# Sbte/RAILS

Measured on AMD Instinct MI355X. Metric: RAILS iterations/sec (+ A*V SpMM HBM GB/s in roofline), m=1M rows/GPU, k=128, fp64, higher is better.
Workload: dtype f64

## Files before the change

### include/rails_hip.h

```cpp
#ifndef RAILS_HIP_H
#define RAILS_HIP_H

#include <stddef.h>
#include <stdint.h>

#ifdef __cplusplus
extern "C" {
#endif

#define RAILS_OK 0
#define RAILS_EINVAL -1
#define RAILS_EHIP -2
#define RAILS_ENOMEM -3
#define RAILS_ELAPACK -4
#define RAILS_ECOMM -5
#define RAILS_ENODEV -6

typedef struct rails_ctx rails_ctx;
typedef struct rails_csr rails_csr;
typedef struct rails_panel rails_panel;

const char *rails_last_error(void);
const char *rails_version(void);

// ... 85 lines not shown

typedef struct rails_sweep_plan rails_sweep_plan;
int rails_sweep_plan_create(int64_t m, int64_t ncols, const int64_t *rowptr, const int32_t *col, const double *val,
                            const int *params, rails_sweep_plan **out);
int rails_sweep_plan_destroy(rails_sweep_plan *plan);
int rails_sweep_plan_info(const rails_sweep_plan *plan, int64_t *iinfo, double *dinfo);
int rails_sweep_plan_array(const rails_sweep_plan *plan, int which, const void **ptr, int64_t *count);


int rails_panel_create(rails_ctx *ctx, int64_t m_local, int capacity, rails_panel **out);
int rails_panel_create_ld(rails_ctx *ctx, int64_t m_local, int capacity, int ld, rails_panel **out);
int rails_panel_destroy(rails_panel *P);
int64_t rails_panel_rows(const rails_panel *P);
int rails_panel_capacity(const rails_panel *P);
int rails_panel_ld(const rails_panel *P);
void *rails_panel_device_ptr(const rails_panel *P);
int rails_panel_reserve(rails_ctx *ctx, rails_panel *P, int capacity);

int rails_panel_upload(rails_ctx *ctx, rails_panel *P, int c0, int nc, const double *host, int64_t ldh);
int rails_panel_download(rails_ctx *ctx, const rails_panel *P, int c0, int nc, double *host, int64_t ldh);

int rails_panel_fill(rails_ctx *ctx, rails_panel *P, int c0, int nc, double value);
int rails_panel_scale(rails_ctx *ctx, rails_panel *P, int c0, int nc, double s);
int rails_panel_copy(rails_ctx *ctx, const rails_panel *X, int xc0, int nc, rails_panel *Y, int yc0);
int rails_panel_axpy(rails_ctx *ctx, double alpha, const rails_panel *X, int xc0, int nc, rails_panel *Y,
                     int yc0);
int rails_panel_random(rails_ctx *ctx, rails_panel *P, int c0, int nc);

int rails_gram(rails_ctx *ctx, const rails_panel *X, int xc0, int a, const rails_panel *Y, int yc0, int b,
               double *C_host, int ldc);

int rails_panel_gemm(rails_ctx *ctx, double alpha, const rails_panel *X, int xc0, int k, const double *C_host,
                     int ldc, int r, double beta, rails_panel *Y, int yc0);

int rails_ctx_enable_library_gemm(rails_ctx *ctx);
int rails_ctx_library_gemm_ready(const rails_ctx *ctx);

int rails_deferred_reserve(rails_ctx *ctx, int nslots, int64_t doubles_per_slot);
int rails_gram_deferred(rails_ctx *ctx, const rails_panel *X, int xc0, int a, const rails_panel *Y, int yc0, int b, int slot);
int rails_panel_gemm_deferred(rails_ctx *ctx, double alpha, const rails_panel *X, int xc0, int k, int slot, int ld, int r, double beta,
                              rails_panel *Y, int yc0);
int rails_chol_inverse_deferred(rails_ctx *ctx, int slot_in, int w, int slot_out);
int rails_update_gram_deferred(rails_ctx *ctx, double alpha, const rails_panel *X, int xc0, int k, const double *C_host, int ldc, int r,
                               rails_panel *Y, int yc0, int r2, int slot);
int rails_update_gram_deferred_out(rails_ctx *ctx, double alpha, const rails_panel *X, int xc0, int k, const double *C_host, int ldc, int r,
                                   const rails_panel *Y, int yc0, rails_panel *Yout, int oc0, int r2, int slot);
int rails_deferred_fetch(rails_ctx *ctx, int slot, int64_t n, double *host_out);

int rails_panel_gemm_wide(rails_ctx *ctx, double alpha, const rails_panel *X, int xc0, int k, const double *C_host, int ldc, int r,
                          double beta, rails_panel *Y, int yc0);

void rails_dense_set_tile_fit(int on);
int rails_dense_tile_fit(void);
int rails_dense_last_tiles(const rails_ctx *ctx, int *update_gram_nbw, int *gram_cols_ti, int *gemm_wide_tr);

int rails_orthogonalize(rails_ctx *ctx, rails_panel *V, int k_old, int w, int method, int *used);
int rails_orthogonalize_deflated(rails_ctx *ctx, rails_panel *V, int k_old, int w, const rails_panel *N, int nc0, int q, int method, int *used);

int rails_panel_colnorms2(rails_ctx *ctx, const rails_panel *X, int c0, int nc, double *out_host);

int rails_orthogonalize_range(rails_ctx *ctx, rails_panel *V, int k_old, int w, const rails_panel *N, int nc0, int q, double tol, int *kept,
                              int32_t *kept_idx);

int rails_resid_lanczos(rails_ctx *ctx, const rails_panel *AV, int avc0, const rails_panel *MV, int mvc0, int k,
                        const double *T_host, int ldt, const rails_panel *B, int bc0, int p, int L,
                        double *H_host, int ldh, int *steps);

int rails_resid_lanczos_sparse(rails_ctx *ctx, const rails_panel *AV, int avc0, const rails_panel *MV, int mvc0, int k, const double *T_host,
                               int ldt, const rails_sprhs *S, int L, double *H_host, int ldh, int *steps);

int rails_lanczos_start(rails_ctx *ctx, const rails_panel *AV, int avc0, const rails_panel *MV, int mvc0, int k,
                        const rails_panel *B, int bc0, int p, double *sums_host);

int rails_lanczos_vectors(rails_ctx *ctx, const double *S_host, int lds, int w, rails_panel *Out, int oc0);
int rails_lanczos_last_launch(rails_ctx *ctx, int *nch, int *unroll, int *nblocks);
int rails_lanczos_release(rails_ctx *ctx);

int rails_ctx_reserve_staging(rails_ctx *ctx, size_t bytes);
int rails_timer_start(rails_ctx *ctx);
int rails_timer_stop(rails_ctx *ctx, double *ms);


void rails_sb03md(char dico, char job, char fact, char trans, int n, double *A, int lda, double *X, int ldx,
                  double *scale, int *info);
void rails_sb03md_counts(long *smith, long *schur);
void rails_sb03md_adi_counts(long *extended, long *fresh);
void rails_sb03md_set_pause(int calls);
void rails_dsyev(char jobz, char uplo, int n, double *a, int lda, double *w, int *info);
void rails_dsteqr(char compz, int n, double *d, double *e, double *z, int ldz, double *work, int *info);
void rails_dgemm(char transa, char transb, int m, int n, int k, double alpha, const double *A, int lda, const double *B,
                 int ldb, double beta, double *C, int ldc);
void rails_dtrsm(char side, char uplo, char transa, char diag, int m, int n, double alpha, const double *A, int lda, double *B, int ldb);
void rails_dpotrf(char uplo, int n, double *a, int lda, int *info);
void rails_dpstrf(char uplo, int n, double *a, int lda, int *piv, int *rank, double tol, int *info);
void rails_range_basis(int m, int n, double *a, int lda, double tol, double *q, int ldq, int *rank, int *info);
int rails_host_lapack_init(const char *path);
const char *rails_host_lapack_path(void);

#ifdef __cplusplus
}
#endif
#endif
```

### rails_amd/_lib.py

```python
import ctypes as C
import os

_HERE = os.path.dirname(os.path.abspath(__file__))
LIB_PATH = os.path.join(_HERE, "lib", "librails_hip.so")

_dp = C.POINTER(C.c_double)
_ip = C.POINTER(C.c_int)
_i64p = C.POINTER(C.c_int64)
_i32p = C.POINTER(C.c_int32)
_vp = C.c_void_p

ALLREDUCE_FN = C.CFUNCTYPE(C.c_int, C.c_void_p, C.c_void_p, C.c_size_t, C.c_void_p)
HALO_FN = C.CFUNCTYPE(C.c_int, C.c_void_p, C.c_void_p, C.c_void_p, C.c_int, C.c_void_p)
APPLY_FN = C.CFUNCTYPE(C.c_int, C.c_void_p, C.c_int, C.c_void_p, C.c_int, C.c_int, C.c_void_p, C.c_int)

SIGNATURES = {
    "rails_last_error": (C.c_char_p, []),
    "rails_version": (C.c_char_p, []),
    "rails_ctx_create": (C.c_int, [C.c_int, _vp, C.POINTER(_vp)]),
    "rails_ctx_destroy": (C.c_int, [_vp]),
    "rails_ctx_sync": (C.c_int, [_vp]),
    "rails_ctx_stream": (_vp, [_vp]),
    "rails_ctx_set_meter": (C.c_int, [_vp, C.c_int]),
    "rails_ctx_enable_library_gemm": (C.c_int, [_vp]),
# ... 27 lines not shown
    "rails_csr_sweep_stats": (C.c_int, [_vp, C.c_int, _dp]),
    "rails_csr_tile_stats": (C.c_int, [_vp, _dp]),
    "rails_csr_prepare": (C.c_int, [_vp, _vp, C.c_int, C.c_int, C.POINTER(C.c_int)]),
    "rails_csr_last_kernel": (C.c_char_p, [_vp]),
    "rails_sweep_plan_create": (C.c_int, [C.c_int64, C.c_int64, _i64p, _i32p, _dp, _ip, C.POINTER(_vp)]),
    "rails_sweep_plan_destroy": (C.c_int, [_vp]),
    "rails_sweep_plan_info": (C.c_int, [_vp, _i64p, _dp]),
    "rails_sweep_plan_array": (C.c_int, [_vp, C.c_int, C.POINTER(_vp), _i64p]),
    "rails_panel_create": (C.c_int, [_vp, C.c_int64, C.c_int, C.POINTER(_vp)]),
    "rails_panel_create_ld": (C.c_int, [_vp, C.c_int64, C.c_int, C.c_int, C.POINTER(_vp)]),
    "rails_panel_destroy": (C.c_int, [_vp]),
    "rails_panel_rows": (C.c_int64, [_vp]),
    "rails_panel_capacity": (C.c_int, [_vp]),
    "rails_panel_ld": (C.c_int, [_vp]),
    "rails_panel_device_ptr": (_vp, [_vp]),
    "rails_panel_reserve": (C.c_int, [_vp, _vp, C.c_int]),
    "rails_panel_upload": (C.c_int, [_vp, _vp, C.c_int, C.c_int, _dp, C.c_int64]),
    "rails_panel_download": (C.c_int, [_vp, _vp, C.c_int, C.c_int, _dp, C.c_int64]),
    "rails_panel_fill": (C.c_int, [_vp, _vp, C.c_int, C.c_int, C.c_double]),
    "rails_panel_scale": (C.c_int, [_vp, _vp, C.c_int, C.c_int, C.c_double]),
    "rails_panel_copy": (C.c_int, [_vp, _vp, C.c_int, C.c_int, _vp, C.c_int]),
    "rails_panel_axpy": (C.c_int, [_vp, C.c_double, _vp, C.c_int, C.c_int, _vp, C.c_int]),
    "rails_sptrsv_create": (C.c_int, [_vp, C.c_int64, _i64p, _i32p, _dp, C.c_int, C.c_int, C.POINTER(_vp)]),
    "rails_sptrsv_destroy": (None, [_vp]),
    "rails_sptrsv_levels": (C.c_int64, [_vp]),
    "rails_sptrsv_solve": (C.c_int, [_vp, _vp, _vp, C.c_int, C.c_int]),
    "rails_panel_permute_rows": (C.c_int, [_vp, _vp, C.c_int, C.c_int, _vp, C.c_int, _vp, C.c_int]),
    "rails_index_upload": (C.c_int, [_vp, _i32p, C.c_int64, C.POINTER(_vp)]),
    "rails_index_free": (None, [_vp, _vp]),
    "rails_lu_create": (C.c_int, [_vp, C.c_int64, _i64p, _i32p, _dp, _i64p, _i32p, _dp, _i32p, _i32p, _i32p, C.c_int64, C.POINTER(_vp)]),
    "rails_lu_destroy": (None, [_vp]),
    "rails_lu_solve": (C.c_int, [_vp, _vp, C.c_int, _vp, C.c_int, C.c_int, _vp, C.c_int]),
    "rails_lu_stats": (C.c_int, [_vp, _i64p, C.c_int]),
    "rails_csr_create_lu": (C.c_int, [_vp, _vp, C.POINTER(_vp)]),
    "rails_csr_transpose_host": (C.c_int, [C.c_int64, C.c_int64, _i64p, _i32p, _dp, _i64p, _i32p, _dp]),
    "rails_csr_gram_norm2_host": (C.c_int, [C.c_int64, C.c_int64, _i64p, _i32p, _dp, _i64p, _i32p, _dp, _dp]),
    "rails_sprhs_create": (C.c_int, [_vp, C.c_int64, C.c_int, _i64p, _i32p, _dp, C.POINTER(_vp)]),
    "rails_sprhs_destroy": (None, [_vp]),
    "rails_sprhs_rows": (C.c_int64, [_vp]),
    "rails_sprhs_cols": (C.c_int64, [_vp]),
    "rails_sprhs_nnz": (C.c_int64, [_vp]),
    "rails_sprhs_gram_norm2": (C.c_double, [_vp]),
    "rails_sprhs_apply": (C.c_int, [_vp, _vp, C.c_int, _vp, C.c_int, C.c_int, _vp, C.c_int]),
    "rails_csr_create_sprhs": (C.c_int, [_vp, _vp, C.POINTER(_vp)]),
    "rails_csr_cols": (C.c_int64, [_vp]),
    "rails_csr_sprhs": (_vp, [_vp]),
    "rails_resid_lanczos_sparse": (C.c_int, [_vp, _vp, C.c_int, _vp, C.c_int, C.c_int, _dp, C.c_int, _vp, C.c_int, _dp, C.c_int, _ip]),
    "rails_panel_random": (C.c_int, [_vp, _vp, C.c_int, C.c_int]),
    "rails_gram": (C.c_int, [_vp, _vp, C.c_int, C.c_int, _vp, C.c_int, C.c_int, _dp, C.c_int]),
    "rails_panel_gemm": (C.c_int, [_vp, C.c_double, _vp, C.c_int, C.c_int, _dp, C.c_int, C.c_int, C.c_double, _vp, C.c_int]),
    "rails_panel_gemm_wide": (C.c_int, [_vp, C.c_double, _vp, C.c_int, C.c_int, _dp, C.c_int, C.c_int, C.c_double, _vp, C.c_int]),
    "rails_dense_set_tile_fit": (None, [C.c_int]),
    "rails_dense_tile_fit": (C.c_int, []),
    "rails_dense_last_tiles": (C.c_int, [_vp, _ip, _ip, _ip]),
    "rails_orthogonalize": (C.c_int, [_vp, _vp, C.c_int, C.c_int, C.c_int, _ip]),
    "rails_orthogonalize_deflated": (C.c_int, [_vp, _vp, C.c_int, C.c_int, _vp, C.c_int, C.c_int, C.c_int, _ip]),
    "rails_panel_colnorms2": (C.c_int, [_vp, _vp, C.c_int, C.c_int, _dp]),
    "rails_orthogonalize_range": (C.c_int, [_vp, _vp, C.c_int, C.c_int, _vp, C.c_int, C.c_int, C.c_double, _ip, _i32p]),
    "rails_resid_lanczos": (C.c_int, [_vp, _vp, C.c_int, _vp, C.c_int, C.c_int, _dp, C.c_int, _vp, C.c_int, C.c_int, C.c_int,
                                      _dp, C.c_int, _ip]),
    "rails_lanczos_start": (C.c_int, [_vp, _vp, C.c_int, _vp, C.c_int, C.c_int, _vp, C.c_int, C.c_int, _dp]),
    "rails_lanczos_vectors": (C.c_int, [_vp, _dp, C.c_int, C.c_int, _vp, C.c_int]),
    "rails_lanczos_last_launch": (C.c_int, [_vp, _ip, _ip, _ip]),
    "rails_lanczos_release": (C.c_int, [_vp]),
    "rails_timer_start": (C.c_int, [_vp]),
    "rails_timer_stop": (C.c_int, [_vp, _dp]),
    "rails_sb03md": (None, [C.c_char, C.c_char, C.c_char, C.c_char, C.c_int, _dp, C.c_int, _dp, C.c_int, _dp, _ip]),
    "rails_dsyev": (None, [C.c_char, C.c_char, C.c_int, _dp, C.c_int, _dp, _ip]),
    "rails_dsteqr": (None, [C.c_char, C.c_int, _dp, _dp, _dp, C.c_int, _dp, _ip]),
    "rails_ctx_reserve_staging": (C.c_int, [_vp, C.c_size_t]),
    "rails_sb03md_set_pause": (None, [C.c_int]),
    "rails_sb03md_counts": (None, [C.POINTER(C.c_long), C.POINTER(C.c_long)]),
    "rails_sb03md_adi_counts": (None, [C.POINTER(C.c_long), C.POINTER(C.c_long)]),
    "rails_dtrsm": (None, [C.c_char, C.c_char, C.c_char, C.c_char, C.c_int, C.c_int, C.c_double, _dp, C.c_int, _dp, C.c_int]),
    "rails_dgemm": (None, [C.c_char, C.c_char, C.c_int, C.c_int, C.c_int, C.c_double, _dp, C.c_int, _dp, C.c_int, C.c_double, _dp, C.c_int]),
    "rails_dpotrf": (None, [C.c_char, C.c_int, _dp, C.c_int, _ip]),
    "rails_dpstrf": (None, [C.c_char, C.c_int, _dp, C.c_int, _ip, _ip, C.c_double, _ip]),
    "rails_range_basis": (None, [C.c_int, C.c_int, _dp, C.c_int, C.c_double, _dp, C.c_int, _ip, _ip]),
    "rails_host_lapack_init": (C.c_int, [C.c_char_p]),
    "rails_host_lapack_path": (C.c_char_p, []),
}

_lib = None


class RailsError(RuntimeError):
    pass


def load():
    global _lib
    if _lib is not None:
        return _lib
    if not os.path.exists(LIB_PATH):
        raise RailsError(
            "rails_amd: %s is missing -- build it with `python -c 'import __graft_entry__ as g; g.build()'` "
            "or `make -C rails_amd/csrc`; there is no CPU fallback" % LIB_PATH)
    lib = C.CDLL(LIB_PATH, mode=C.RTLD_GLOBAL)
    for name, (res, args) in SIGNATURES.items():
        fn = getattr(lib, name)
        fn.restype = res
        fn.argtypes = args
    try:
        from ._solver_sigs import bind as _bind_solver
        _bind_solver(lib)
    except ImportError:
# ... 13 lines not shown
```

### rails_amd/csrc/dense.hip

```cpp
#include "rails_internal.h"

#include <dlfcn.h>
#include <atomic>
#include <mutex>

#include <algorithm>

namespace {

typedef double v4f64 __attribute__((ext_vector_type(4)));
typedef double v2f64 __attribute__((ext_vector_type(2)));

std::atomic<int> g_tile_fit{-1};

bool dense_tile_fit()
{
    int v = g_tile_fit.load(std::memory_order_relaxed);
    if (v < 0) {
        const char *e = getenv("RAILS_DENSE_TILE_FIT");
        int undecided = -1;
        g_tile_fit.compare_exchange_strong(undecided, (e ? atoi(e) : 1) ? 1 : 0);
        v = g_tile_fit.load(std::memory_order_relaxed);
    }
    return v != 0;
}

__device__ __forceinline__ v4f64 mfma_f64(double a, double b, v4f64 c)
{
    return __builtin_amdgcn_mfma_f64_16x16x4f64(a, b, c, 0, 0, 0);
}

struct OneSeg {
    const double *X;
    int ld;
    struct Row {
        const double *x;
    };
    __device__ int col(int c) const { return c; }
    __device__ Row row(int64_t r) const { return {X + r * ld}; }
    __device__ static const double *at(Row r, int c) { return r.x + c; }
};
struct TwoSeg {
    const double *X1;
    int ld1, a1;
    const double *X2;
    int ld2;
    struct Col {
        int off;
        bool second;
    };
    struct Row {
        const double *x1, *x2;
    };
    __device__ Col col(int c) const
    {
        const bool second = c >= a1;
        return {second ? c - a1 : c, second};
    }
    __device__ Row row(int64_t r) const { return {X1 + r * ld1, X2 + r * ld2}; }
    __device__ static const double *at(Row r, Col c) { return (c.second ? r.x2 : r.x1) + c.off; }
};

template <int TI, int TJ>
__global__ __launch_bounds__(256) __attribute__((amdgpu_waves_per_eu(3, 8))) void k_gram(const double *__restrict__ X, int ldx, int a, const double *__restrict__ Y, int ldy,
                                              int b, int64_t m, int64_t rows_per_slab, int ngj, double *__restrict__ partial)
{
    const OneSeg Xo{X, ldx};
#include "dense_gram.inc"
}

template <int TI, int TJ>
__global__ __launch_bounds__(256) void k_gram2(const double *__restrict__ X1, int ldx1, int a1, const double *__restrict__ X2, int ldx2, int a,
                                               const double *__restrict__ Y, int ldy, int b, int64_t m, int64_t rows_per_slab, int ngj,
                                               double *__restrict__ partial)
{
    const TwoSeg Xo{X1, ldx1, a1, X2, ldx2};
#include "dense_gram.inc"
}

template <int TI, int TJ, int NE = 0>
__global__ __launch_bounds__(256) __attribute__((amdgpu_waves_per_eu(3, 8))) void k_gram_cols(const double *__restrict__ X, int ldx, int a,
                                                                                             const double *__restrict__ Y, int ldy, int b, int64_t m,
                                                                                             int64_t rows_per_slab, double *__restrict__ partial)
{
    const OneSeg Xo{X, ldx};
#include "dense_gram_cols.inc"
}

template <int TI, int TJ, int NE>
__global__ __launch_bounds__(256) void k_gram_cols2(const double *__restrict__ X1, int ldx1, int a1, const double *__restrict__ X2, int ldx2, int a,
                                                    const double *__restrict__ Y, int ldy, int b, int64_t m, int64_t rows_per_slab,
                                                    double *__restrict__ partial)
{
    const TwoSeg Xo{X1, ldx1, a1, X2, ldx2};
#include "dense_gram_cols.inc"
}

__global__ __launch_bounds__(1024) void k_reduce_partials(const double *__restrict__ partial, int64_t nslab, int64_t n, double *__restrict__ out)
{
    __shared__ double sh[16][64];
    const int tx = threadIdx.x & 63, ty = threadIdx.x >> 6;
    const int64_t e = (int64_t)blockIdx.x * 64 + tx;
    double s = 0.0;
    if (e < n)
        for (int64_t t = ty; t < nslab; t += 16) s += partial[t * n + e];
    sh[ty][tx] = s;
    __syncthreads();
    if (ty == 0 && e < n) {
        double r = 0.0;
#pragma unroll
        for (int g = 0; g < 16; ++g) r += sh[g][tx];
        out[e] = r;
    }
}

template <int TI, int TJ>
void launch_gram(rails_ctx *c, const double *X, int ldx, int a, const double *Y, int ldy, int b, int64_t m, int64_t rps,
                 int64_t nslab, double *partial)
{
    int ngi = (a + 16 * TI - 1) / (16 * TI), ngj = (b + 16 * TJ - 1) / (16 * TJ);
    RAILS_LAUNCH((k_gram<TI, TJ>), dim3((unsigned)nslab, (unsigned)(ngi * ngj)), dim3(256), 0, c->stream, X, ldx, a, Y, ldy, b,
                       m, rps, ngj, partial);
}

template <int TI, int TJ>
void launch_gram2(rails_ctx *c, const double *X1, int ldx1, int a1, const double *X2, int ldx2, int a, const double *Y, int ldy, int b, int64_t m,
                  int64_t rps, int64_t nslab, double *partial)
{
    int ngi = (a + 16 * TI - 1) / (16 * TI), ngj = (b + 16 * TJ - 1) / (16 * TJ);
    RAILS_LAUNCH((k_gram2<TI, TJ>), dim3((unsigned)nslab, (unsigned)(ngi * ngj)), dim3(256), 0, c->stream, X1, ldx1, a1, X2, ldx2, a, Y, ldy, b,
                 m, rps, ngj, partial);
}

template <int TR, int KC>
__global__ __launch_bounds__(256) void k_panel_gemm(double alpha, const double *X, int ldx, int k,
                                                    const double *__restrict__ C, int r, double beta, double *Yp,
                                                    int ldy, int64_t m, int vec_ok)
{
    const OneSeg Xo{X, ldx};
#define RAILS_PG_VEC4(c) (vec_ok && (c) + 4 <= k)
#include "dense_panel_gemm.inc"
}

template <int TR, int KC>
__global__ __launch_bounds__(256) void k_panel_gemm2(double alpha, const double *X1, int ldx1, int a1, const double *X2, int ldx2, int a,
                                                     const double *__restrict__ C, int r, double beta, double *Yp, int ldy, int64_t m, int vec1,
                                                     int vec2)
{
    const TwoSeg Xo{X1, ldx1, a1, X2, ldx2};
    const int k = a;
#define RAILS_PG_VEC4(c) (((c) + 4 <= a1 && vec1) || ((c) >= a1 && (c) + 4 <= a && vec2))
#include "dense_panel_gemm.inc"
}

template <int TR, int KC>
void launch_pg(rails_ctx *c, double alpha, const double *X, int ldx, int k, const double *C, int r, double beta, double *Y,
               int ldy, int64_t m, int vec_ok)
{
    int64_t grid = (m + 63) / 64;
    RAILS_LAUNCH((k_panel_gemm<TR, KC>), dim3((unsigned)grid), dim3(256), 0, c->stream, alpha, X, ldx, k, C, r, beta, Y,
                       ldy, m, vec_ok);
}

__global__ void k_pack_ct(const double *__restrict__ C, int k, int r, int kpad, int RL, double *__restrict__ out)
{
    const int64_t n = (int64_t)kpad * RL;
    for (int64_t q = (int64_t)blockIdx.x * blockDim.x + threadIdx.x; q < n; q += (int64_t)gridDim.x * blockDim.x) {
        const int kl = (int)(q / RL), j = (int)(q % RL);
        out[q] = (kl < k && j < r) ? C[kl + (int64_t)j * k] : 0.0;
    }
}

template <int TR>
__global__ __launch_bounds__(512) void k_panel_gemm_wide(double alpha, const double *__restrict__ X, int ldx, int k, const double *__restrict__ Ct ,
                                                         int r, double beta, double *__restrict__ Yp, int ldy, int64_t m, int vec_ok, int skip_tail)
{
    constexpr int KC = 32, RL = 16 * TR + 4, CHUNK_B = KC * RL * 8, PIECES = CHUNK_B / 1024;
    static_assert(CHUNK_B % 1024 == 0, "whole LDS-DMA pieces per chunk");
    extern __shared__ double Cs[];
    const int lane = threadIdx.x & 63;
    const int wave = __builtin_amdgcn_readfirstlane((int)(threadIdx.x >> 6));
    const int li = lane & 15, kk = lane >> 4;
    const int64_t r0 = ((int64_t)blockIdx.x * 8 + wave) * 16;
    const int64_t myrow = r0 + li;
// ... 105 lines not shown
}

int gram_cols_tiles(int ntiles, bool one_tile)
{
    const int cand2[3] = {3, 4, 5}, cand1[3] = {4, 6, 8};
    const int *cand = one_tile ? cand1 : cand2;
    int best = cand[1], best_cost = 1 << 30;
    for (int q = 0; q < 3; ++q) {
        int ti = cand[q], strips = (ntiles + ti - 1) / ti, cost = (strips + 3) / 4 * 4 * ti;
        if (cost < best_cost) best = ti, best_cost = cost;
    }
    if (one_tile && best == 6 && (ntiles + 4) / 5 == (ntiles + 5) / 6 && dense_tile_fit()) best = 5;
    return best;
}

#define RAILS_GRAM_COLS_CASE(K, TI, TJ, NE, ...) RAILS_LAUNCH((K<TI, TJ, NE>), grid, dim3(256), 0, c->stream, __VA_ARGS__, Y, ldy, b, m, rps, c->ws)
#define RAILS_GRAM_COLS(K, ...)                                                                                                            \
    do {                                                                                                                                   \
        const int ntiles = (a + 15) / 16, best = gram_cols_tiles(ntiles, b <= 16 || extra);                                                \
        const dim3 grid((unsigned)nslab, (unsigned)(((ntiles + best - 1) / best + 3) / 4));                                                \
        c->last_gram_cols_ti = best;                                                                                                       \
        if (extra) {                                                                                                                       \
            if (best == 4)                                                                                                                 \
                RAILS_GRAM_COLS_CASE(K, 4, 1, 1, __VA_ARGS__);                                                                             \
            else if (best == 5)                                                                                                            \
                RAILS_GRAM_COLS_CASE(K, 5, 1, 1, __VA_ARGS__);                                                                             \
            else if (best == 6)                                                                                                            \
                RAILS_GRAM_COLS_CASE(K, 6, 1, 1, __VA_ARGS__);                                                                             \
            else                                                                                                                           \
                RAILS_GRAM_COLS_CASE(K, 8, 1, 1, __VA_ARGS__);                                                                             \
        } else if (b <= 16) {                                                                                                              \
            if (best == 4)                                                                                                                 \
                RAILS_GRAM_COLS_CASE(K, 4, 1, 0, __VA_ARGS__);                                                                             \
            else if (best == 5)                                                                                                            \
                RAILS_GRAM_COLS_CASE(K, 5, 1, 0, __VA_ARGS__);                                                                             \
            else if (best == 6)                                                                                                            \
                RAILS_GRAM_COLS_CASE(K, 6, 1, 0, __VA_ARGS__);                                                                             \
            else                                                                                                                           \
                RAILS_GRAM_COLS_CASE(K, 8, 1, 0, __VA_ARGS__);                                                                             \
        } else if (best == 3)                                                                                                              \
            RAILS_GRAM_COLS_CASE(K, 3, 2, 0, __VA_ARGS__);                                                                                 \
        else if (best == 4)                                                                                                                \
            RAILS_GRAM_COLS_CASE(K, 4, 2, 0, __VA_ARGS__);                                                                                 \
        else                                                                                                                               \
            RAILS_GRAM_COLS_CASE(K, 5, 2, 0, __VA_ARGS__);                                                                                 \
    } while (0)

}

extern "C" void rails_dense_set_tile_fit(int on) { g_tile_fit.store(on ? 1 : 0); }

extern "C" int rails_dense_tile_fit(void) { return dense_tile_fit() ? 1 : 0; }

extern "C" int rails_dense_last_tiles(const rails_ctx *c, int *update_gram_nbw, int *gram_cols_ti, int *gemm_wide_tr)
{
    RAILS_REQUIRE(c, "rails_dense_last_tiles: null context");
    if (update_gram_nbw) *update_gram_nbw = c->last_update_gram_nbw;
    if (gram_cols_ti) *gram_cols_ti = c->last_gram_cols_ti;
    if (gemm_wide_tr) *gemm_wide_tr = c->last_gemm_wide_tr;
    return RAILS_OK;
}

int rails_gram_dev(rails_ctx *c, const double *X, int ldx, const double *Y, int ldy, int64_t m, int a, int b, double *C_dev)
{
    if (a <= 0 || b <= 0) return RAILS_OK;
    int64_t nslab, rps;
    gram_slabs(m, a, b, &nslab, &rps);
    size_t n = (size_t)a * b;
    RAILS_TRY(rails_ws_reserve(c, (size_t)nslab * n * sizeof(double)));
    if (b <= 16 && a <= 16)
        launch_gram<1, 1>(c, X, ldx, a, Y, ldy, b, m, rps, nslab, c->ws);
    else if (b <= 32 && a >= 128) {
        static const int cols_form = getenv("RAILS_GRAM_COLS") ? atoi(getenv("RAILS_GRAM_COLS")) : 1;
        if (cols_form) {
            static const int extra_env = getenv("RAILS_GRAM_EXTRA_COLUMN") ? atoi(getenv("RAILS_GRAM_EXTRA_COLUMN")) : 1;
            const bool extra = extra_env && b == 17;
            RAILS_GRAM_COLS(k_gram_cols, X, ldx, a);
        } else if (b <= 16)
            launch_gram<8, 1>(c, X, ldx, a, Y, ldy, b, m, rps, nslab, c->ws);
        else
            launch_gram<4, 2>(c, X, ldx, a, Y, ldy, b, m, rps, nslab, c->ws);
    } else if (b <= 16)
        launch_gram<8, 1>(c, X, ldx, a, Y, ldy, b, m, rps, nslab, c->ws);
    else if (a <= 16)
        launch_gram<1, 8>(c, X, ldx, a, Y, ldy, b, m, rps, nslab, c->ws);
    else if (a <= 32 && b <= 32)
        launch_gram<2, 2>(c, X, ldx, a, Y, ldy, b, m, rps, nslab, c->ws);
    else if (b <= 32)
        launch_gram<4, 2>(c, X, ldx, a, Y, ldy, b, m, rps, nslab, c->ws);
    else if (a <= 32)
        launch_gram<2, 4>(c, X, ldx, a, Y, ldy, b, m, rps, nslab, c->ws);
    else
        launch_gram<2, 4>(c, X, ldx, a, Y, ldy, b, m, rps, nslab, c->ws);
    RAILS_LAUNCH(k_reduce_partials, dim3((unsigned)((n + 63) / 64)), dim3(1024), 0, c->stream, c->ws, nslab, (int64_t)n, C_dev);
    RAILS_HIP_CHECK(hipGetLastError());
    return RAILS_OK;
}

int rails_gram2_dev(rails_ctx *c, const double *X1, int ldx1, int a1, const double *X2, int ldx2, int a2, const double *Y, int ldy, int64_t m, int b,
                    double *C_dev)
{
    const int a = a1 + a2;
    if (a <= 0 || b <= 0) return RAILS_OK;
    int64_t nslab, rps;
    gram_slabs(m, a, b, &nslab, &rps);
    const size_t n = (size_t)a * b;
    RAILS_TRY(rails_ws_reserve(c, (size_t)nslab * n * sizeof(double)));
    if (a >= 128 && b <= 32) {
        const bool extra = b == 17;
        RAILS_GRAM_COLS(k_gram_cols2, X1, ldx1, a1, X2, ldx2, a);
    } else if (a <= 16 && b <= 16)
        launch_gram2<1, 1>(c, X1, ldx1, a1, X2, ldx2, a, Y, ldy, b, m, rps, nslab, c->ws);
    else if (b <= 16)
        launch_gram2<8, 1>(c, X1, ldx1, a1, X2, ldx2, a, Y, ldy, b, m, rps, nslab, c->ws);
    else
        launch_gram2<4, 2>(c, X1, ldx1, a1, X2, ldx2, a, Y, ldy, b, m, rps, nslab, c->ws);
    RAILS_LAUNCH(k_reduce_partials, dim3((unsigned)((n + 63) / 64)), dim3(1024), 0, c->stream, c->ws, nslab, (int64_t)n, C_dev);
    RAILS_HIP_CHECK(hipGetLastError());
    return RAILS_OK;
}

extern "C" int rails_gram(rails_ctx *c, const rails_panel *X, int xc0, int a, const rails_panel *Y, int yc0, int b, double *C_host,
                          int ldc)
{
    if (c) hipSetDevice(c->device);
    rails_slow_guard slow__(c, "rails_gram", a, b);
    RAILS_REQUIRE(c && X && Y, "rails_gram: null argument");
    RAILS_REQUIRE(a >= 0 && b >= 0 && xc0 >= 0 && yc0 >= 0 && xc0 + a <= X->cap && yc0 + b <= Y->cap,
                  "rails_gram: windows [%d,%d) / [%d,%d) outside capacities %d / %d", xc0, xc0 + a, yc0, yc0 + b, X->cap, Y->cap);
    RAILS_REQUIRE(X->m == Y->m, "rails_gram: row mismatch %lld vs %lld", (long long)X->m, (long long)Y->m);
    RAILS_REQUIRE(a == 0 || b == 0 || (C_host && ldc >= a), "rails_gram: bad output buffer (ldc %d < %d)", ldc, a);
    if (a == 0 || b == 0) return RAILS_OK;
    size_t n = (size_t)a * b;
    RAILS_TRY(rails_small_reserve(c, n * sizeof(double)));
    RAILS_TRY(rails_pinned_reserve(c, n * sizeof(double)));
    if (X->m > 0)
        RAILS_TRY(rails_gram_dev(c, X->d + xc0, X->ld, Y->d + yc0, Y->ld, X->m, a, b, c->small));
    else
        RAILS_HIP_CHECK(hipMemsetAsync(c->small, 0, n * sizeof(double), c->stream));
    RAILS_TRY(rails_allreduce_dev(c, c->small, n));
    RAILS_HIP_CHECK(hipMemcpyAsync(c->pinned, c->small, n * sizeof(double), hipMemcpyDeviceToHost, c->stream));
    RAILS_HIP_CHECK(rails_stream_sync(c));
    for (int j = 0; j < b; ++j) memcpy(C_host + (size_t)j * ldc, c->pinned + (size_t)j * a, sizeof(double) * a);
    return RAILS_OK;
}

namespace {

__global__ __launch_bounds__(256) void k_colnorms2(const double *__restrict__ X, int ldx, int nc, int64_t m, int64_t rows_per_slab, int tx_bits,
                                                   int vec_ok, double *__restrict__ partial)
{
    __shared__ double sh[256][2];
    const int TX = 1 << tx_bits, TY = 256 >> tx_bits;
    const int tx = threadIdx.x & (TX - 1), ty = threadIdx.x >> tx_bits;
    const int c = 2 * tx;
    const bool has0 = c < nc, has1 = c + 1 < nc;
    const int64_t r_begin = (int64_t)blockIdx.x * rows_per_slab;
    const int64_t r_end = r_begin + rows_per_slab < m ? r_begin + rows_per_slab : m;
    double s0[4] = {0.0, 0.0, 0.0, 0.0}, s1[4] = {0.0, 0.0, 0.0, 0.0};
    if (has0) {
        const bool pair = has1 && vec_ok;
        auto load = [&](int64_t r, double &a, double &b) {
            const double *src = X + r * ldx + c;
            if (pair) {
                const v2f64 t = *reinterpret_cast<const v2f64 *>(src);
                a = t.x;
                b = t.y;
            } else {
                a = src[0];
                b = has1 ? src[1] : 0.0;
// ... 5 lines not shown
#pragma unroll
            for (int s = 0; s < 4; ++s) load(r + s * (int64_t)TY, a[s], b[s]);
#pragma unroll
            for (int s = 0; s < 4; ++s) {
                s0[s] += a[s] * a[s];
                s1[s] += b[s] * b[s];
            }
        }
#pragma unroll
        for (int s = 0; s < 3; ++s)
            if (r + s * (int64_t)TY < r_end) {
                double a, b;
                load(r + s * (int64_t)TY, a, b);
                s0[s] += a * a;
                s1[s] += b * b;
            }
    }
    sh[threadIdx.x][0] = ((s0[0] + s0[1]) + s0[2]) + s0[3];
    sh[threadIdx.x][1] = ((s1[0] + s1[1]) + s1[2]) + s1[3];
    __syncthreads();
    for (int half = TY >> 1; half > 0; half >>= 1) {
        if (ty < half) {
            sh[threadIdx.x][0] += sh[threadIdx.x + (half << tx_bits)][0];
            sh[threadIdx.x][1] += sh[threadIdx.x + (half << tx_bits)][1];
        }
        __syncthreads();
    }
    if (ty == 0 && has0) {
        double *dst = partial + (int64_t)blockIdx.x * nc + c;
        dst[0] = sh[tx][0];
        if (has1) dst[1] = sh[tx][1];
    }
}

}

int rails_colnorms2_dev(rails_ctx *c, const double *X, int ldx, int64_t m, int nc, double *out_dev)
{
    if (nc <= 0) return RAILS_OK;
    if (m <= 0) {
        RAILS_HIP_CHECK(hipMemsetAsync(out_dev, 0, (size_t)nc * sizeof(double), c->stream));
        return RAILS_OK;
    }
    const int pairs = (nc + 1) / 2;
    int tx_bits = 0;
    while ((1 << tx_bits) < pairs) ++tx_bits;
    const int TY = 256 >> tx_bits;
    int64_t nslab = std::max<int64_t>(1, std::min<int64_t>(1024, m / ((int64_t)TY * 8)));
    const int64_t rps = (m + nslab - 1) / nslab;
    nslab = (m + rps - 1) / rps;
    RAILS_TRY(rails_ws_reserve(c, (size_t)nslab * nc * sizeof(double)));
    const int vec_ok = ((((uintptr_t)X) & 15) == 0 && (ldx % 2) == 0) ? 1 : 0;
    RAILS_LAUNCH(k_colnorms2, dim3((unsigned)nslab), dim3(256), 0, c->stream, X, ldx, nc, m, rps, tx_bits, vec_ok, c->ws);
    RAILS_LAUNCH(k_reduce_partials, dim3((unsigned)((nc + 63) / 64)), dim3(1024), 0, c->stream, c->ws, nslab, (int64_t)nc, out_dev);
    RAILS_HIP_CHECK(hipGetLastError());
    return RAILS_OK;
}

extern "C" int rails_panel_colnorms2(rails_ctx *c, const rails_panel *X, int c0, int nc, double *out_host)
{
    if (c) hipSetDevice(c->device);
    RAILS_REQUIRE(c && X, "rails_panel_colnorms2: null argument");
    RAILS_REQUIRE(c0 >= 0 && nc >= 0 && c0 + nc <= X->cap, "rails_panel_colnorms2: window [%d,%d) outside capacity %d", c0, c0 + nc, X->cap);
    RAILS_REQUIRE(nc == 0 || out_host, "rails_panel_colnorms2: null output buffer");
    if (nc == 0) return RAILS_OK;
    RAILS_TRY(rails_small_reserve(c, (size_t)nc * sizeof(double)));
    RAILS_TRY(rails_pinned_reserve(c, (size_t)nc * sizeof(double)));
    for (int j0 = 0; j0 < nc; j0 += 512)
        RAILS_TRY(rails_colnorms2_dev(c, X->d + c0 + j0, X->ld, X->m, std::min(512, nc - j0), c->small + j0));
    RAILS_TRY(rails_allreduce_dev(c, c->small, (size_t)nc));
    RAILS_HIP_CHECK(hipMemcpyAsync(c->pinned, c->small, (size_t)nc * sizeof(double), hipMemcpyDeviceToHost, c->stream));
    RAILS_HIP_CHECK(rails_stream_sync(c));
    memcpy(out_host, c->pinned, (size_t)nc * sizeof(double));
    return RAILS_OK;
}


namespace {

__global__ void k_compact_cols(const double *__restrict__ src, int ld, int k, int r, double *__restrict__ dst)
{
    const int64_t n = (int64_t)k * r;
    for (int64_t q = (int64_t)blockIdx.x * blockDim.x + threadIdx.x; q < n; q += (int64_t)gridDim.x * blockDim.x) dst[q] = src[(q / k) * ld + (q % k)];
}

__global__ __launch_bounds__(64) void k_small_chol(const double *__restrict__ G, int w, double *__restrict__ M)
{
    constexpr int LD = 49;
    __shared__ double S[48 * LD], Ri[48 * LD], d[48];
    const int t = threadIdx.x;
    const bool mine = t < w;
    for (int q = t; q < w * w; q += 64) S[(q / w) * LD + (q % w)] = G[q];
    __syncthreads();
    if (mine) d[t] = sqrt(S[t * LD + t]);
    __syncthreads();
    for (int q = t; q < w * w; q += 64) S[(q / w) * LD + (q % w)] /= d[q % w] * d[q / w];
    __syncthreads();
    for (int i = 0; i < w; ++i) {
        const double piv = sqrt(S[i * LD + i]);
        double rij = 0.0;
        if (mine && t >= i) rij = (t == i) ? piv : S[t * LD + i] / piv;
        __syncthreads();
        if (mine && t >= i) S[t * LD + i] = rij;
        __syncthreads();
        if (mine && t > i)
            for (int l = i + 1; l <= t; ++l) S[t * LD + l] -= S[l * LD + i] * rij;
        __syncthreads();
// ... 201 lines not shown
                               double *Yo, int ldo, int r2, int64_t m, int64_t ntiles)
{
    if (ne == 0)
        RAILS_LAUNCH((k_update_gram<NBW, 0>), dim3(grid), dim3(256), 0, c->stream, alpha, X, ldx, k, C, r, Y, ldy, Yo, ldo, r2, m, ntiles, c->ws);
    else
        RAILS_LAUNCH((k_update_gram<NBW, 1>), dim3(grid), dim3(256), 0, c->stream, alpha, X, ldx, k, C, r, Y, ldy, Yo, ldo, r2, m, ntiles, c->ws);
    c->last_update_gram_nbw = NBW;
}

extern "C" int rails_update_gram_deferred_out(rails_ctx *c, double alpha, const rails_panel *X, int xc0, int k, const double *C_host, int ldc, int r,
                                              const rails_panel *Y, int yc0, rails_panel *Yout, int oc0, int r2, int slot)
{
    if (c) hipSetDevice(c->device);
    rails_slow_guard slow__(c, "rails_update_gram_deferred", k, r);
    RAILS_REQUIRE(c && X && Y && Yout && C_host, "rails_update_gram_deferred: null argument");
    RAILS_REQUIRE(k >= 1 && r >= 1 && r <= 256 && r2 >= 1 && r2 <= r && ldc >= k && xc0 >= 0 && yc0 >= 0 && xc0 + k <= X->cap && yc0 + r <= Y->cap && X->m == Y->m,
                  "rails_update_gram_deferred: bad shapes");
    RAILS_REQUIRE(oc0 >= 0 && oc0 + r <= Yout->cap && Yout->m == X->m, "rails_update_gram_deferred: output window [%d,%d) outside capacity %d, or row mismatch", oc0,
                  oc0 + r, Yout->cap);
    if (X->d == Y->d) RAILS_REQUIRE(xc0 + k <= yc0 || yc0 + r <= xc0, "rails_update_gram_deferred: overlapping windows of one panel");
    if (X->d == Yout->d) RAILS_REQUIRE(xc0 + k <= oc0 || oc0 + r <= xc0, "rails_update_gram_deferred: overlapping windows of one panel");
    if (Y->d == Yout->d) RAILS_REQUIRE(yc0 == oc0 || yc0 + r <= oc0 || oc0 + r <= yc0, "rails_update_gram_deferred: partially overlapping windows of one panel");
    const size_t n = (size_t)k * r2;
    RAILS_SLOT_CHECK(slot, n, "rails_update_gram_deferred");
    double *out = c->defer_dev + (size_t)slot * c->defer_slot;
    if (X->m == 0) {
        RAILS_HIP_CHECK(hipMemsetAsync(out, 0, n * sizeof(double), c->stream));
    } else {
        const size_t nc = (size_t)k * r;
        RAILS_TRY(rails_small_reserve(c, nc * sizeof(double)));
        RAILS_TRY(rails_pinned_begin_write(c, nc * sizeof(double)));
        for (int j = 0; j < r; ++j) memcpy(c->pinned + (size_t)j * k, C_host + (size_t)j * ldc, sizeof(double) * k);
        RAILS_HIP_CHECK(hipMemcpyAsync(c->small, c->pinned, nc * sizeof(double), hipMemcpyHostToDevice, c->stream));
        RAILS_TRY(rails_pinned_end_write(c));
        static const int fused_env = getenv("RAILS_FUSED_UPDATE_GRAM") ? atoi(getenv("RAILS_FUSED_UPDATE_GRAM")) : 1;
        const double *Xp = X->d + xc0;
        const double *Ypp = Y->d + yc0;
        double *Yop = Yout->d + oc0;
        const int k4 = (k + 3) & ~3;
        const bool rows_ok = ((((uintptr_t)Xp) & 15) == 0 && (X->ld % 2) == 0) && (k4 == k || (X->d == Y->d && yc0 == xc0 + k && r >= k4 - k));
        if (fused_env && rows_ok && r <= 17 && r2 <= 16 && k >= 32 && k <= 512 && X->m >= 4096) {
            const int64_t ntiles = (X->m + 15) / 16;
            const unsigned grid = (unsigned)std::min<int64_t>(ntiles, 2 * (int64_t)std::max(c->num_cu, 1));
            const int ne = r > 16 ? r - 16 : 0;
            RAILS_TRY(rails_ws_reserve(c, (size_t)grid * n * sizeof(double)));
            if (k <= 256)
                launch_update_gram<4>(c, ne, grid, alpha, Xp, X->ld, k, c->small, r, Ypp, Y->ld, Yop, Yout->ld, r2, X->m, ntiles);
            else if (k <= 320 && dense_tile_fit())
                launch_update_gram<5>(c, ne, grid, alpha, Xp, X->ld, k, c->small, r, Ypp, Y->ld, Yop, Yout->ld, r2, X->m, ntiles);
            else if (k <= 384)
                launch_update_gram<6>(c, ne, grid, alpha, Xp, X->ld, k, c->small, r, Ypp, Y->ld, Yop, Yout->ld, r2, X->m, ntiles);
            else
                launch_update_gram<8>(c, ne, grid, alpha, Xp, X->ld, k, c->small, r, Ypp, Y->ld, Yop, Yout->ld, r2, X->m, ntiles);
            RAILS_LAUNCH(k_reduce_partials, dim3((unsigned)((n + 63) / 64)), dim3(1024), 0, c->stream, c->ws, (int64_t)grid, (int64_t)n, out);
            RAILS_HIP_CHECK(hipGetLastError());
            c->n_update_gram_fused++;
        } else {
            if (Yop != Ypp) RAILS_TRY(rails_panel_copy(c, Y, yc0, r, Yout, oc0));
            RAILS_TRY(rails_panel_gemm_dev(c, alpha, Xp, X->ld, k, c->small, r, 1.0, Yop, Yout->ld, X->m));
            RAILS_TRY(rails_gram_dev(c, Xp, X->ld, Yop, Yout->ld, X->m, k, r2, out));
        }
    }
    RAILS_TRY(rails_allreduce_dev(c, out, n));
    RAILS_HIP_CHECK(hipMemcpyAsync(c->defer_pin + (size_t)slot * c->defer_slot, out, n * sizeof(double), hipMemcpyDeviceToHost, c->stream));
    return RAILS_OK;
}

extern "C" int rails_update_gram_deferred(rails_ctx *c, double alpha, const rails_panel *X, int xc0, int k, const double *C_host, int ldc, int r,
                                          rails_panel *Y, int yc0, int r2, int slot)
{
    return rails_update_gram_deferred_out(c, alpha, X, xc0, k, C_host, ldc, r, Y, yc0, Y, yc0, r2, slot);
}

extern "C" int rails_chol_inverse_deferred(rails_ctx *c, int slot_in, int w, int slot_out)
{
    if (c) hipSetDevice(c->device);
    RAILS_REQUIRE(c && w >= 1 && w <= 48 && slot_in != slot_out, "rails_chol_inverse_deferred: bad argument (w = %d)", w);
    RAILS_SLOT_CHECK(slot_in, (size_t)w * w, "rails_chol_inverse_deferred");
    RAILS_SLOT_CHECK(slot_out, (size_t)w * w, "rails_chol_inverse_deferred");
    RAILS_LAUNCH(k_small_chol, dim3(1), dim3(64), 0, c->stream, c->defer_dev + (size_t)slot_in * c->defer_slot, w, c->defer_dev + (size_t)slot_out * c->defer_slot);
    RAILS_HIP_CHECK(hipGetLastError());
    RAILS_HIP_CHECK(hipMemcpyAsync(c->defer_pin + (size_t)slot_out * c->defer_slot, c->defer_dev + (size_t)slot_out * c->defer_slot, (size_t)w * w * sizeof(double),
                                   hipMemcpyDeviceToHost, c->stream));
    return RAILS_OK;
}

extern "C" int rails_deferred_fetch(rails_ctx *c, int slot, int64_t n, double *host_out)
{
    RAILS_REQUIRE(host_out && n >= 0, "rails_deferred_fetch: bad argument");
    RAILS_SLOT_CHECK(slot, n, "rails_deferred_fetch");
    memcpy(host_out, c->defer_pin + (size_t)slot * c->defer_slot, (size_t)n * sizeof(double));
    return RAILS_OK;
}

int rails_panel_gemm_dev(rails_ctx *c, double alpha, const double *X, int ldx, int k, const double *C_dev, int r, double beta,
                         double *Y, int ldy, int64_t m)
{
    if (r <= 0 || m <= 0) return RAILS_OK;
    int vec_ok = ((((uintptr_t)X) & 15) == 0 && (ldx % 2) == 0) ? 1 : 0;
    int tr = (r + 15) / 16;
    if (tr <= 1)
        launch_pg<1, 32>(c, alpha, X, ldx, k, C_dev, r, beta, Y, ldy, m, vec_ok);
    else if (tr <= 2)
        launch_pg<2, 32>(c, alpha, X, ldx, k, C_dev, r, beta, Y, ldy, m, vec_ok);
    else if (tr <= 4)
        launch_pg<4, 32>(c, alpha, X, ldx, k, C_dev, r, beta, Y, ldy, m, vec_ok);
    else if (tr <= 8)
// ... 186 lines not shown
```

### rails_amd/csrc/dense_gram.inc

```
    __shared__ double red[TI * TJ * 256];
    const int lane = threadIdx.x & 63;
    const int wave = threadIdx.x >> 6;
    const int li = lane & 15, kk = lane >> 4;
    const int gi = blockIdx.y / ngj, gj = blockIdx.y % ngj;
    const int xcol0 = gi * TI * 16, ycol0 = gj * TJ * 16;
    const int64_t r_begin = (int64_t)blockIdx.x * rows_per_slab;
    int64_t r_end = r_begin + rows_per_slab;
    if (r_end > m) r_end = m;

    v4f64 acc[TI][TJ];
#pragma unroll
    for (int i = 0; i < TI; ++i)
#pragma unroll
        for (int j = 0; j < TJ; ++j) acc[i][j] = (v4f64){0.0, 0.0, 0.0, 0.0};

    decltype(Xo.col(0)) xcol[TI];
    int yoff[TJ];
#pragma unroll
    for (int i = 0; i < TI; ++i) xcol[i] = Xo.col((xcol0 + 16 * i + li) < a ? xcol0 + 16 * i + li : 0);
#pragma unroll
    for (int j = 0; j < TJ; ++j) yoff[j] = (ycol0 + 16 * j + li) < b ? ycol0 + 16 * j + li : 0;

    auto fetch = [&](int64_t r, double *xa, double *yb) {
        const int64_t row = r + kk;
        const bool rok = row < r_end;
        const int64_t rc = rok ? row : (r_end > 0 ? r_end - 1 : 0);
        const auto xr = Xo.row(rc);
        const double *yr = Y + rc * ldy;
#pragma unroll
        for (int i = 0; i < TI; ++i) xa[i] = *Xo.at(xr, xcol[i]);
#pragma unroll
        for (int j = 0; j < TJ; ++j) {
            const double t = yr[yoff[j]];
            yb[j] = rok ? t : 0.0;
        }
    };
    double xa[TI], yb[TJ], xn[TI], yn[TJ];
    int64_t r = r_begin + 4 * wave;
    if (r < r_end) fetch(r, xa, yb);
    for (; r < r_end; r += 16) {
        const bool more = r + 16 < r_end;
        if (more) fetch(r + 16, xn, yn);
#pragma unroll
        for (int i = 0; i < TI; ++i)
#pragma unroll
            for (int j = 0; j < TJ; ++j) acc[i][j] = mfma_f64(xa[i], yb[j], acc[i][j]);
        if (more) {
#pragma unroll
            for (int i = 0; i < TI; ++i) xa[i] = xn[i];
#pragma unroll
            for (int j = 0; j < TJ; ++j) yb[j] = yn[j];
        }
    }

    for (int w = 1; w < 4; ++w) {
        if (wave == w) {
#pragma unroll
            for (int i = 0; i < TI; ++i)
#pragma unroll
                for (int j = 0; j < TJ; ++j)
#pragma unroll
                    for (int v = 0; v < 4; ++v) red[((i * TJ + j) * 4 + v) * 64 + lane] = acc[i][j][v];
        }
        __syncthreads();
        if (wave == 0) {
#pragma unroll
            for (int i = 0; i < TI; ++i)
#pragma unroll
                for (int j = 0; j < TJ; ++j)
#pragma unroll
                    for (int v = 0; v < 4; ++v) acc[i][j][v] += red[((i * TJ + j) * 4 + v) * 64 + lane];
        }
        __syncthreads();
    }
    if (wave == 0) {
        double *P = partial + (int64_t)blockIdx.x * a * b;
#pragma unroll
        for (int i = 0; i < TI; ++i)
#pragma unroll
            for (int j = 0; j < TJ; ++j)
#pragma unroll
                for (int v = 0; v < 4; ++v) {
                    int ci = xcol0 + 16 * i + kk + 4 * v;
                    int cj = ycol0 + 16 * j + li;
                    if (ci < a && cj < b) P[ci + (int64_t)cj * a] = acc[i][j][v];
                }
    }
```

Measured before the change: 238.9.

## Deepen gram kernel load pipeline and add unrolled partial-reduction kernel

Adds a templated prefetch depth to the gram kernel, enabled by default at depth 4 for small tiles (TI+TJ<=4). The kernel keeps D rows-groups of X/Y loads in flight ahead of the MFMA accumulation instead of double buffering, to hide HBM latency. It also replaces the partial-sum reduction with a 256-thread kernel that issues 16 unrolled loads per thread before summing, which raises memory-level parallelism. Both paths are selectable through environment variables or setters. The cost is more registers per thread, which may lower occupancy, plus extra tail handling.

Measured after the change: 243.3 (median of 6 runs). About the same (+1.9%).

```diff
diff --git a/include/rails_hip.h b/include/rails_hip.h
--- a/include/rails_hip.h
+++ b/include/rails_hip.h
@@ -161,6 +161,10 @@
 
 void rails_dense_set_tile_fit(int on);
 int rails_dense_tile_fit(void);
+void rails_dense_set_gram_depth(int depth);
+int rails_dense_gram_depth(void);
+void rails_dense_set_reduce_form(int form);
+int rails_dense_reduce_form(void);
 int rails_dense_last_tiles(const rails_ctx *ctx, int *update_gram_nbw, int *gram_cols_ti, int *gemm_wide_tr);
 
 int rails_orthogonalize(rails_ctx *ctx, rails_panel *V, int k_old, int w, int method, int *used);
diff --git a/rails_amd/_lib.py b/rails_amd/_lib.py
--- a/rails_amd/_lib.py
+++ b/rails_amd/_lib.py
@@ -103,6 +103,10 @@
     "rails_panel_gemm_wide": (C.c_int, [_vp, C.c_double, _vp, C.c_int, C.c_int, _dp, C.c_int, C.c_int, C.c_double, _vp, C.c_int]),
     "rails_dense_set_tile_fit": (None, [C.c_int]),
     "rails_dense_tile_fit": (C.c_int, []),
+    "rails_dense_set_gram_depth": (None, [C.c_int]),
+    "rails_dense_gram_depth": (C.c_int, []),
+    "rails_dense_set_reduce_form": (None, [C.c_int]),
+    "rails_dense_reduce_form": (C.c_int, []),
     "rails_dense_last_tiles": (C.c_int, [_vp, _ip, _ip, _ip]),
     "rails_orthogonalize": (C.c_int, [_vp, _vp, C.c_int, C.c_int, C.c_int, _ip]),
     "rails_orthogonalize_deflated": (C.c_int, [_vp, _vp, C.c_int, C.c_int, _vp, C.c_int, C.c_int, C.c_int, _ip]),
diff --git a/rails_amd/csrc/dense.hip b/rails_amd/csrc/dense.hip
--- a/rails_amd/csrc/dense.hip
+++ b/rails_amd/csrc/dense.hip
@@ -21,6 +21,35 @@
         int undecided = -1;
         g_tile_fit.compare_exchange_strong(undecided, (e ? atoi(e) : 1) ? 1 : 0);
         v = g_tile_fit.load(std::memory_order_relaxed);
+    }
+    return v != 0;
+}
+
+constexpr int kGramDepthDefault = 4;
+std::atomic<int> g_gram_depth{-1}, g_reduce_form{-1};
+
+int gram_depth_supported(int d) { return d >= 2 ? kGramDepthDefault : 1; }
+
+int dense_gram_depth()
+{
+    int v = g_gram_depth.load(std::memory_order_relaxed);
+    if (v < 0) {
+        const char *e = getenv("RAILS_DENSE_GRAM_DEPTH");
+        int undecided = -1;
+        g_gram_depth.compare_exchange_strong(undecided, gram_depth_supported(e ? atoi(e) : kGramDepthDefault));
+        v = g_gram_depth.load(std::memory_order_relaxed);
+    }
+    return v;
+}
+
+bool dense_reduce_form()
+{
+    int v = g_reduce_form.load(std::memory_order_relaxed);
+    if (v < 0) {
+        const char *e = getenv("RAILS_DENSE_REDUCE_FORM");
+        int undecided = -1;
+        g_reduce_form.compare_exchange_strong(undecided, (e ? atoi(e) : 1) ? 1 : 0);
+        v = g_reduce_form.load(std::memory_order_relaxed);
     }
     return v != 0;
 }
@@ -61,7 +90,7 @@
     __device__ static const double *at(Row r, Col c) { return (c.second ? r.x2 : r.x1) + c.off; }
 };
 
-template <int TI, int TJ>
+template <int TI, int TJ, int D = 1>
 __global__ __launch_bounds__(256) __attribute__((amdgpu_waves_per_eu(3, 8))) void k_gram(const double *__restrict__ X, int ldx, int a, const double *__restrict__ Y, int ldy,
                                               int b, int64_t m, int64_t rows_per_slab, int ngj, double *__restrict__ partial)
 {
@@ -69,7 +98,7 @@
 #include "dense_gram.inc"
 }
 
-template <int TI, int TJ>
+template <int TI, int TJ, int D = 1>
 __global__ __launch_bounds__(256) void k_gram2(const double *__restrict__ X1, int ldx1, int a1, const double *__restrict__ X2, int ldx2, int a,
                                                const double *__restrict__ Y, int ldy, int b, int64_t m, int64_t rows_per_slab, int ngj,
                                                double *__restrict__ partial)
@@ -114,13 +143,64 @@
     }
 }
 
+constexpr int RU = 16;
+__global__ __launch_bounds__(256) void k_reduce_partials_ahead(const double *__restrict__ partial, int64_t nslab, int64_t n, double *__restrict__ out)
+{
+    __shared__ double sh[16][16];
+    const int tx = threadIdx.x & 15, ty = threadIdx.x >> 4;
+    const int64_t e = (int64_t)blockIdx.x * 16 + tx;
+    double s = 0.0;
+    if (e < n) {
+        int64_t t = ty;
+        double v[RU];
+        for (; t + 16 * (RU - 1) < nslab; t += 16 * RU) {
+#pragma unroll
+            for (int u = 0; u < RU; ++u) v[u] = partial[(t + 16 * u) * n + e];
+#pragma unroll
+            for (int u = 0; u < RU; ++u) s += v[u];
+        }
+        if (t < nslab) {
+#pragma unroll
+            for (int u = 0; u < RU; ++u) v[u] = partial[(t + 16 * u < nslab ? t + 16 * u : t) * n + e];
+#pragma unroll
+            for (int u = 0; u < RU; ++u)
+                if (t + 16 * u < nslab) s += v[u];
+        }
+    }
+    sh[ty][tx] = s;
+    __syncthreads();
+    if (ty == 0 && e < n) {
+        double r = 0.0;
+#pragma unroll
+        for (int g = 0; g < 16; ++g) r += sh[g][tx];
+        out[e] = r;
+    }
+}
+
+void launch_reduce_partials(rails_ctx *c, const double *partial, int64_t nslab, int64_t n, double *out)
+{
+    if (dense_reduce_form())
+        RAILS_LAUNCH(k_reduce_partials_ahead, dim3((unsigned)((n + 15) / 16)), dim3(256), 0, c->stream, partial, nslab, n, out);
+    else
+        RAILS_LAUNCH(k_reduce_partials, dim3((unsigned)((n + 63) / 64)), dim3(1024), 0, c->stream, partial, nslab, n, out);
+}
+
+template <int TI, int TJ>
+constexpr bool gram_deep = TI + TJ <= 4;
+
 template <int TI, int TJ>
 void launch_gram(rails_ctx *c, const double *X, int ldx, int a, const double *Y, int ldy, int b, int64_t m, int64_t rps,
                  int64_t nslab, double *partial)
 {
     int ngi = (a + 16 * TI - 1) / (16 * TI), ngj = (b + 16 * TJ - 1) / (16 * TJ);
-    RAILS_LAUNCH((k_gram<TI, TJ>), dim3((unsigned)nslab, (unsigned)(ngi * ngj)), dim3(256), 0, c->stream, X, ldx, a, Y, ldy, b,
-                       m, rps, ngj, partial);
+    const dim3 grid((unsigned)nslab, (unsigned)(ngi * ngj));
+    if constexpr (gram_deep<TI, TJ>) {
+        if (dense_gram_depth() > 1) {
+            RAILS_LAUNCH((k_gram<TI, TJ, kGramDepthDefault>), grid, dim3(256), 0, c->stream, X, ldx, a, Y, ldy, b, m, rps, ngj, partial);
+            return;
+        }
+    }
+    RAILS_LAUNCH((k_gram<TI, TJ, 1>), grid, dim3(256), 0, c->stream, X, ldx, a, Y, ldy, b, m, rps, ngj, partial);
 }
 
 template <int TI, int TJ>
@@ -128,8 +208,14 @@
                   int64_t rps, int64_t nslab, double *partial)
 {
     int ngi = (a + 16 * TI - 1) / (16 * TI), ngj = (b + 16 * TJ - 1) / (16 * TJ);
-    RAILS_LAUNCH((k_gram2<TI, TJ>), dim3((unsigned)nslab, (unsigned)(ngi * ngj)), dim3(256), 0, c->stream, X1, ldx1, a1, X2, ldx2, a, Y, ldy, b,
-                 m, rps, ngj, partial);
+    const dim3 grid((unsigned)nslab, (unsigned)(ngi * ngj));
+    if constexpr (gram_deep<TI, TJ>) {
+        if (dense_gram_depth() > 1) {
+            RAILS_LAUNCH((k_gram2<TI, TJ, kGramDepthDefault>), grid, dim3(256), 0, c->stream, X1, ldx1, a1, X2, ldx2, a, Y, ldy, b, m, rps, ngj, partial);
+            return;
+        }
+    }
+    RAILS_LAUNCH((k_gram2<TI, TJ, 1>), grid, dim3(256), 0, c->stream, X1, ldx1, a1, X2, ldx2, a, Y, ldy, b, m, rps, ngj, partial);
 }
 
 template <int TR, int KC>
@@ -341,6 +427,14 @@
 
 extern "C" int rails_dense_tile_fit(void) { return dense_tile_fit() ? 1 : 0; }
 
+extern "C" void rails_dense_set_gram_depth(int depth) { g_gram_depth.store(gram_depth_supported(depth)); }
+
+extern "C" int rails_dense_gram_depth(void) { return dense_gram_depth(); }
+
+extern "C" void rails_dense_set_reduce_form(int form) { g_reduce_form.store(form ? 1 : 0); }
+
+extern "C" int rails_dense_reduce_form(void) { return dense_reduce_form() ? 1 : 0; }
+
 extern "C" int rails_dense_last_tiles(const rails_ctx *c, int *update_gram_nbw, int *gram_cols_ti, int *gemm_wide_tr)
 {
     RAILS_REQUIRE(c, "rails_dense_last_tiles: null context");
@@ -381,7 +475,7 @@
         launch_gram<2, 4>(c, X, ldx, a, Y, ldy, b, m, rps, nslab, c->ws);
     else
         launch_gram<2, 4>(c, X, ldx, a, Y, ldy, b, m, rps, nslab, c->ws);
-    RAILS_LAUNCH(k_reduce_partials, dim3((unsigned)((n + 63) / 64)), dim3(1024), 0, c->stream, c->ws, nslab, (int64_t)n, C_dev);
+    launch_reduce_partials(c, c->ws, nslab, (int64_t)n, C_dev);
     RAILS_HIP_CHECK(hipGetLastError());
     return RAILS_OK;
 }
@@ -404,7 +498,7 @@
         launch_gram2<8, 1>(c, X1, ldx1, a1, X2, ldx2, a, Y, ldy, b, m, rps, nslab, c->ws);
     else
         launch_gram2<4, 2>(c, X1, ldx1, a1, X2, ldx2, a, Y, ldy, b, m, rps, nslab, c->ws);
-    RAILS_LAUNCH(k_reduce_partials, dim3((unsigned)((n + 63) / 64)), dim3(1024), 0, c->stream, c->ws, nslab, (int64_t)n, C_dev);
+    launch_reduce_partials(c, c->ws, nslab, (int64_t)n, C_dev);
     RAILS_HIP_CHECK(hipGetLastError());
     return RAILS_OK;
 }
@@ -516,7 +610,7 @@
     RAILS_TRY(rails_ws_reserve(c, (size_t)nslab * nc * sizeof(double)));
     const int vec_ok = ((((uintptr_t)X) & 15) == 0 && (ldx % 2) == 0) ? 1 : 0;
     RAILS_LAUNCH(k_colnorms2, dim3((unsigned)nslab), dim3(256), 0, c->stream, X, ldx, nc, m, rps, tx_bits, vec_ok, c->ws);
-    RAILS_LAUNCH(k_reduce_partials, dim3((unsigned)((nc + 63) / 64)), dim3(1024), 0, c->stream, c->ws, nslab, (int64_t)nc, out_dev);
+    launch_reduce_partials(c, c->ws, nslab, (int64_t)nc, out_dev);
     RAILS_HIP_CHECK(hipGetLastError());
     return RAILS_OK;
 }
@@ -824,7 +918,7 @@
                 launch_update_gram<6>(c, ne, grid, alpha, Xp, X->ld, k, c->small, r, Ypp, Y->ld, Yop, Yout->ld, r2, X->m, ntiles);
             else
                 launch_update_gram<8>(c, ne, grid, alpha, Xp, X->ld, k, c->small, r, Ypp, Y->ld, Yop, Yout->ld, r2, X->m, ntiles);
-            RAILS_LAUNCH(k_reduce_partials, dim3((unsigned)((n + 63) / 64)), dim3(1024), 0, c->stream, c->ws, (int64_t)grid, (int64_t)n, out);
+            launch_reduce_partials(c, c->ws, (int64_t)grid, (int64_t)n, out);
             RAILS_HIP_CHECK(hipGetLastError());
             c->n_update_gram_fused++;
         } else {
diff --git a/rails_amd/csrc/dense_gram.inc b/rails_amd/csrc/dense_gram.inc
--- a/rails_amd/csrc/dense_gram.inc
+++ b/rails_amd/csrc/dense_gram.inc
@@ -35,21 +35,47 @@
             yb[j] = rok ? t : 0.0;
         }
     };
-    double xa[TI], yb[TJ], xn[TI], yn[TJ];
-    int64_t r = r_begin + 4 * wave;
-    if (r < r_end) fetch(r, xa, yb);
-    for (; r < r_end; r += 16) {
-        const bool more = r + 16 < r_end;
-        if (more) fetch(r + 16, xn, yn);
+    if constexpr (D == 1) {
+        double xa[TI], yb[TJ], xn[TI], yn[TJ];
+        int64_t r = r_begin + 4 * wave;
+        if (r < r_end) fetch(r, xa, yb);
+        for (; r < r_end; r += 16) {
+            const bool more = r + 16 < r_end;
+            if (more) fetch(r + 16, xn, yn);
 #pragma unroll
-        for (int i = 0; i < TI; ++i)
+            for (int i = 0; i < TI; ++i)
 #pragma unroll
-            for (int j = 0; j < TJ; ++j) acc[i][j] = mfma_f64(xa[i], yb[j], acc[i][j]);
-        if (more) {
+                for (int j = 0; j < TJ; ++j) acc[i][j] = mfma_f64(xa[i], yb[j], acc[i][j]);
+            if (more) {
 #pragma unroll
-            for (int i = 0; i < TI; ++i) xa[i] = xn[i];
+                for (int i = 0; i < TI; ++i) xa[i] = xn[i];
 #pragma unroll
-            for (int j = 0; j < TJ; ++j) yb[j] = yn[j];
+                for (int j = 0; j < TJ; ++j) yb[j] = yn[j];
+            }
+        }
+    } else {
+        double xq[D][TI], yq[D][TJ];
+        int64_t r = r_begin + 4 * wave;
+#pragma unroll
+        for (int d = 0; d < D; ++d) fetch(r + 16 * d, xq[d], yq[d]);
+        for (; r + 16 * (D - 1) < r_end; r += 16 * D) {
+#pragma unroll
+            for (int d = 0; d < D; ++d) {
+#pragma unroll
+                for (int i = 0; i < TI; ++i)
+#pragma unroll
+                    for (int j = 0; j < TJ; ++j) acc[i][j] = mfma_f64(xq[d][i], yq[d][j], acc[i][j]);
+                fetch(r + 16 * (D + d), xq[d], yq[d]);
+            }
+        }
+#pragma unroll
+        for (int d = 0; d < D - 1; ++d) {
+            if (r + 16 * d < r_end) {
+#pragma unroll
+                for (int i = 0; i < TI; ++i)
+#pragma unroll
+                    for (int j = 0; j < TJ; ++j) acc[i][j] = mfma_f64(xq[d][i], yq[d][j], acc[i][j]);
+            }
         }
     }
 
```
